# InternRobotics/InternNav

Measured on AMD Instinct MI355X. Metric: policy steps/sec/node, higher is better.
Workload: dtype bf16

## Files before the change

### internnav_amd/build.py

```python
from __future__ import annotations

import os
import subprocess
import sys
from concurrent.futures import ThreadPoolExecutor
from pathlib import Path

ROOT = Path(__file__).resolve().parent
CSRC = ROOT / "csrc"
OBJ = CSRC / "build"
LIB = ROOT / "libinternnav_amd.so"
ARCH = "gfx950"
FLAGS = ["-O3", "-std=c++17", "-fPIC", f"--offload-arch={ARCH}", "-fno-gpu-rdc", "-Wall", "-Wno-unused-function",
         "-ffp-contract=fast"]


def _sources():
    return sorted(list(CSRC.glob("*.hip")) + list(CSRC.glob("*.cpp")))


def _headers():
    return list(CSRC.glob("*.h")) + list((ROOT.parent / "include").glob("*.h"))


def _stale(target: Path, deps) -> bool:
    if not target.exists():
        return True
    t = target.stat().st_mtime
    return any(d.stat().st_mtime > t for d in deps)


def _compile(src: Path, verbose: bool) -> Path:
    obj = OBJ / (src.name + ".o")
    if _stale(obj, [src] + _headers()):
        cmd = ["hipcc", *FLAGS, "-x", "hip", "-c", str(src), "-o", str(obj)]
        if verbose:
            print(" ".join(cmd), flush=True)
        r = subprocess.run(cmd, capture_output=True, text=True)
        if r.returncode != 0:
            raise RuntimeError(f"hipcc failed for {src.name}:\n{r.stdout}\n{r.stderr}")
        if verbose and r.stderr.strip():
            print(r.stderr, file=sys.stderr)
    return obj


def build(verbose: bool = True) -> Path:
    OBJ.mkdir(parents=True, exist_ok=True)
    srcs = _sources()
    with ThreadPoolExecutor(max_workers=min(8, os.cpu_count() or 1)) as ex:
        objs = list(ex.map(lambda s: _compile(s, verbose), srcs))
    if _stale(LIB, objs):
        cmd = ["hipcc", "-shared", "-fPIC", f"--offload-arch={ARCH}", "-fno-gpu-rdc", *map(str, objs), "-o", str(LIB)]
        if verbose:
            print(" ".join(cmd), flush=True)
        r = subprocess.run(cmd, capture_output=True, text=True)
        if r.returncode != 0:
            raise RuntimeError(f"link failed:\n{r.stdout}\n{r.stderr}")
    return LIB


if __name__ == "__main__":
    print(build())
```

### internnav_amd/csrc/attention.hip

```cpp
#include "common.h"
#include "kernels.h"

namespace {

__device__ __forceinline__ int vt_pos(int kv_local) {
    int sub = kv_local >> 5, w = kv_local & 31;
    int t = w >> 4, x = w & 15;
    return (sub << 5) + ((x >> 2) << 3) + (x & 3) + (t << 2);
}

template <int DP, int DV, int NW, int KVB, bool DROP = false>
__global__ __launch_bounds__(NW * 64) void attn_fwd_kernel(AttnArgs p) {
    constexpr int NT = NW * 64;
    constexpr int KS_LD = DP + 8;
    constexpr int VT_LD = KVB + 8;
    constexpr int KCPR = DP / 8;
    constexpr int VCPR = DV / 8;
    constexpr int NKK = DP / 32;
    constexpr int NST = KVB / 16;
    constexpr int NSB = KVB / 32;
    constexpr int NDT = DV / 16;
    __shared__ __attribute__((aligned(16))) bf16 Ks[KVB * KS_LD];
    __shared__ __attribute__((aligned(16))) bf16 Vt[DV * VT_LD];

// ... 187 lines not shown
    f32x4 acc_o[NDT];
#pragma unroll
    for (int i = 0; i < NDT; ++i) acc_o[i] = f32x4{0.f, 0.f, 0.f, 0.f};
    if (kv0 < len_k) {
        bf16x8 qf[NKK];
#pragma unroll
        for (int kk = 0; kk < NKK; ++kk) {
            int d = kk * 32 + g * 8;
            qf[kk] = (live && d < p.D) ? *reinterpret_cast<const bf16x8*>(Q + d) : zero8;
        }
        constexpr int NKI = KVB * KCPR / 64, NVI = KVB * VCPR / 64;
        static_assert((KVB * KCPR) % 64 == 0 && (KVB * VCPR) % 64 == 0, "chunk pieces must divide evenly over the wave");
        bf16x8 kreg[NKI], vreg[NVI];
#pragma unroll
        for (int u = 0; u < NKI; ++u) {
            const int q = lane + u * 64, row = q / KCPR, c = q % KCPR, kv = kv0 + row;
            kreg[u] = (kv < len_k && c * 8 < p.D) ? *reinterpret_cast<const bf16x8*>(K + (size_t)kv * p.k_rs + c * 8) : zero8;
        }
#pragma unroll
        for (int u = 0; u < NVI; ++u) {
            const int q = lane + u * 64, row = q / VCPR, c = q % VCPR, kv = kv0 + row;
            vreg[u] = (kv < len_k) ? *reinterpret_cast<const bf16x8*>(V + (size_t)kv * p.v_rs + c * 8) : zero8;
        }
#pragma unroll
        for (int u = 0; u < NKI; ++u) {
            const int q = lane + u * 64, row = q / KCPR, c = q % KCPR;
            *reinterpret_cast<bf16x8*>(&Ks[row * KS_LD + c * 8]) = kreg[u];
        }
#pragma unroll
        for (int u = 0; u < NVI; ++u) {
            const int q = lane + u * 64, row = q / VCPR, c = q % VCPR;
            const int pos = vt_pos(row);
#pragma unroll
            for (int i = 0; i < 8; ++i) Vt[(c * 8 + i) * VT_LD + ((pos + 8 * c) & (KVB - 1))] = vreg[u][i];
        }
        __syncthreads();
        f32x4 s[NST];
#pragma unroll
        for (int t = 0; t < NST; ++t) {
            s[t] = f32x4{0.f, 0.f, 0.f, 0.f};
#pragma unroll
            for (int kk = 0; kk < NKK; ++kk) {
                bf16x8 kf = *reinterpret_cast<const bf16x8*>(&Ks[(t * 16 + lq) * KS_LD + kk * 32 + g * 8]);
                s[t] = __builtin_amdgcn_mfma_f32_16x16x32_bf16(kf, qf[kk], s[t], 0, 0, 0);
            }
        }
        const float sc = p.scale * 1.4426950408889634f;
        const int causal_shift = len_k - p.Lq;
        float mx = -INFINITY;
#pragma unroll
        for (int t = 0; t < NST; ++t)
#pragma unroll
            for (int r = 0; r < 4; ++r) {
                int kv = kv0 + t * 16 + g * 4 + r;
                bool ok = live && (kv < len_k) && (!p.causal || kv <= qpos + causal_shift);
                float v = ok ? s[t][r] * sc : -INFINITY;
                s[t][r] = v;
                mx = fmaxf(mx, v);
            }
        mx = fmaxf(mx, __shfl_xor(mx, 16));
        mx = fmaxf(mx, __shfl_xor(mx, 32));
        m_run = mx;
        const float m_use = (mx == -INFINITY) ? 0.f : mx;
        float rs = 0.f;
#pragma unroll
        for (int t = 0; t < NST; ++t)
#pragma unroll
            for (int r = 0; r < 4; ++r) {
                float e = exp2f(s[t][r] - m_use);
                s[t][r] = e;
                rs += e;
            }
        rs += __shfl_xor(rs, 16);
        rs += __shfl_xor(rs, 32);
        l_run = rs;
#pragma unroll
        for (int sb = 0; sb < NSB; ++sb) {
            bf16x8 pf;
#pragma unroll
            for (int r = 0; r < 4; ++r) {
                pf[r] = (bf16)s[2 * sb][r];
                pf[4 + r] = (bf16)s[2 * sb + 1][r];
            }
#pragma unroll
            for (int nt = 0; nt < NDT; ++nt) {
                bf16x8 vf = *reinterpret_cast<const bf16x8*>(&Vt[(nt * 16 + lq) * VT_LD + ((sb * 32 + g * 8 + 8 * ((nt * 16 + lq) >> 3)) & (KVB - 1))]);
                acc_o[nt] = __builtin_amdgcn_mfma_f32_16x16x32_bf16(vf, pf, acc_o[nt], 0, 0, 0);
            }
        }
    }
    float* orow = out + (size_t)lq * (DV + 2);
#pragma unroll
    for (int nt = 0; nt < NDT; ++nt) *reinterpret_cast<f32x4*>(orow + nt * 16 + g * 4) = acc_o[nt];
    if (g == 0) { orow[DV] = m_run; orow[DV + 1] = l_run; }
}

template <int DV>
__global__ __launch_bounds__(64) void attn_decode_combine_kernel(AttnArgs p, const float* __restrict__ ws, int nsplit, int rtiles) {
    const int lane = threadIdx.x;
    const int R = blockIdx.x, kh = blockIdx.y, b = blockIdx.z;
    const int G = p.H / p.Hkv;
    const int rt = R / 16, lq = R % 16;
    const int head = kh * G + R / p.Lq, qpos = R % p.Lq;
    const float* base = ws + (((size_t)b * p.Hkv + kh) * rtiles + rt) * nsplit * (size_t)(16 * (DV + 2)) + (size_t)lq * (DV + 2);
    const size_t sstride = (size_t)16 * (DV + 2);
    float m = -INFINITY;
    for (int s0 = 0; s0 < nsplit; s0 += 64) {
        const int s = s0 + lane;
        m = fmaxf(m, s < nsplit ? base[s * sstride + DV] : -INFINITY);
    }
    m = wave_max(m);
    const float m_use = (m == -INFINITY) ? 0.f : m;
    float l = 0.f, o0 = 0.f, o1 = 0.f;
    for (int s0 = 0; s0 < nsplit; s0 += 64) {
        const int s = s0 + lane;
        const float ms = s < nsplit ? base[s * sstride + DV] : -INFINITY;
        const float wl = (ms == -INFINITY) ? 0.f : exp2f(ms - m_use);
        l += s < nsplit ? base[s * sstride + DV + 1] * wl : 0.f;
        const int cnt = min(64, nsplit - s0);
#pragma unroll 8
        for (int j = 0; j < cnt; ++j) {
            const float w = __shfl(wl, j);
            const float* q = base + (size_t)(s0 + j) * sstride;
            if (lane < DV) o0 += q[lane] * w;
            if (lane + 64 < DV) o1 += q[lane + 64] * w;
        }
    }
    l = wave_sum(l);
    const float inv = l > 0.f ? 1.0f / l : 0.f;
    bf16* O = reinterpret_cast<bf16*>(p.O) + (size_t)b * p.o_bs + (size_t)qpos * p.o_rs + (size_t)head * p.o_hs;
    if (lane < p.D) O[lane] = (bf16)(o0 * inv);
    if (lane + 64 < p.D) O[lane + 64] = (bf16)(o1 * inv);
}

constexpr int DEC_FUSED_WAVES = 4, DEC_FUSED_MAX_CHUNKS = 16;

template <int DP, int DV>
__global__ __launch_bounds__(DEC_FUSED_WAVES * 64) void attn_decode_fused_kernel(AttnArgs p, int nsplit, int rtiles) {
    constexpr int KVB = 64, KS_LD = DP + 8, VT_LD = KVB + 8, KCPR = DP / 8, VCPR = DV / 8, NKK = DP / 32, NST = KVB / 16, NSB = KVB / 32, NDT = DV / 16;
    constexpr int PER_WAVE = KVB * KS_LD + DV * VT_LD;
    constexpr int PLD = DV + 2;
    static_assert(16 * PLD * 4 <= KVB * KS_LD * 2, "the partial of a wave fits its K image");
    extern __shared__ __attribute__((aligned(16))) char dec_smem[];
    const int tid = threadIdx.x, lane = tid & 63, g = lane >> 4, lq = lane & 15;
    const int wave = __builtin_amdgcn_readfirstlane(tid >> 6);
    bf16* Ks = reinterpret_cast<bf16*>(dec_smem) + wave * PER_WAVE;
    bf16* Vt = Ks + KVB * KS_LD;
    const int kh = blockIdx.x / rtiles, rt = blockIdx.x % rtiles, b = blockIdx.y;
    const int G = p.H / p.Hkv;
    const int R = rt * 16 + lq;
    const bool live = R < G * p.Lq;
    const int head = kh * G + (live ? R / p.Lq : 0), qpos = live ? R % p.Lq : 0;
    int len_k = p.Lk;
    if (p.k_len) len_k = min(p.k_len[b], p.Lk);
    const bf16* __restrict__ Q = reinterpret_cast<const bf16*>(p.Q) + (size_t)b * p.q_bs + (size_t)qpos * p.q_rs + (size_t)head * p.q_hs;
    const bf16* __restrict__ K = reinterpret_cast<const bf16*>(p.K) + (size_t)b * p.k_bs + (size_t)kh * p.k_hs;
    const bf16* __restrict__ V = reinterpret_cast<const bf16*>(p.V) + (size_t)b * p.v_bs + (size_t)kh * p.v_hs;
    const bf16x8 zero8 = {0, 0, 0, 0, 0, 0, 0, 0};
    float m_run = -INFINITY, l_run = 0.f;
    f32x4 acc_o[NDT];
#pragma unroll
    for (int i = 0; i < NDT; ++i) acc_o[i] = f32x4{0.f, 0.f, 0.f, 0.f};
    bf16x8 qf[NKK];
#pragma unroll
    for (int kk = 0; kk < NKK; ++kk) {
        const int d = kk * 32 + g * 8;
        qf[kk] = (live && d < p.D) ? *reinterpret_cast<const bf16x8*>(Q + d) : zero8;
    }
    constexpr int NKI = KVB * KCPR / 64, NVI = KVB * VCPR / 64;
    static_assert((KVB * KCPR) % 64 == 0 && (KVB * VCPR) % 64 == 0, "chunk pieces must divide evenly over the wave");
    bf16x8 kreg[NKI], vreg[NVI];
    auto fetch = [&](int kv0) {
#pragma unroll
        for (int u = 0; u < NKI; ++u) {
            const int q = lane + u * 64, row = q / KCPR, c = q % KCPR, kv = kv0 + row;
            kreg[u] = (kv < len_k && c * 8 < p.D) ? *reinterpret_cast<const bf16x8*>(K + (size_t)kv * p.k_rs + c * 8) : zero8;
        }
#pragma unroll
        for (int u = 0; u < NVI; ++u) {
            const int q = lane + u * 64, row = q / VCPR, c = q % VCPR, kv = kv0 + row;
            vreg[u] = (kv < len_k) ? *reinterpret_cast<const bf16x8*>(V + (size_t)kv * p.v_rs + c * 8) : zero8;
        }
    };
    const float sc = p.scale * 1.4426950408889634f;
    const int causal_shift = len_k - p.Lq;
    int split = wave;
    if (split * DEC_CHUNK < len_k) fetch(split * DEC_CHUNK);
    for (; split * DEC_CHUNK < len_k; split += DEC_FUSED_WAVES) {
        const int kv0 = split * DEC_CHUNK;
#pragma unroll
        for (int u = 0; u < NKI; ++u) {
            const int q = lane + u * 64, row = q / KCPR, c = q % KCPR;
            *reinterpret_cast<bf16x8*>(&Ks[row * KS_LD + c * 8]) = kreg[u];
        }
#pragma unroll
        for (int u = 0; u < NVI; ++u) {
            const int q = lane + u * 64, row = q / VCPR, c = q % VCPR;
            const int pos = vt_pos(row);
#pragma unroll
            for (int i = 0; i < 8; ++i) Vt[(c * 8 + i) * VT_LD + ((pos + 8 * c) & (KVB - 1))] = vreg[u][i];
        }
        if ((split + DEC_FUSED_WAVES) * DEC_CHUNK < len_k) fetch((split + DEC_FUSED_WAVES) * DEC_CHUNK);
        asm volatile("s_waitcnt lgkmcnt(0)" ::: "memory");
        __builtin_amdgcn_wave_barrier();
        f32x4 s[NST];
#pragma unroll
        for (int t = 0; t < NST; ++t) {
            s[t] = f32x4{0.f, 0.f, 0.f, 0.f};
#pragma unroll
            for (int kk = 0; kk < NKK; ++kk) {
                bf16x8 kf = *reinterpret_cast<const bf16x8*>(&Ks[(t * 16 + lq) * KS_LD + kk * 32 + g * 8]);
                s[t] = __builtin_amdgcn_mfma_f32_16x16x32_bf16(kf, qf[kk], s[t], 0, 0, 0);
            }
        }
        float mx = -INFINITY;
#pragma unroll
        for (int t = 0; t < NST; ++t)
#pragma unroll
            for (int r = 0; r < 4; ++r) {
                const int kv = kv0 + t * 16 + g * 4 + r;
                const bool ok = live && (kv < len_k) && (!p.causal || kv <= qpos + causal_shift);
                const float v = ok ? s[t][r] * sc : -INFINITY;
                s[t][r] = v;
                mx = fmaxf(mx, v);
            }
        mx = fmaxf(mx, __shfl_xor(mx, 16));
        mx = fmaxf(mx, __shfl_xor(mx, 32));
        const float m_new = fmaxf(m_run, mx);
        const float m_use = (m_new == -INFINITY) ? 0.f : m_new;
        const float alpha = (m_run == -INFINITY) ? 0.f : exp2f(m_run - m_use);
        float rs = 0.f;
#pragma unroll
        for (int t = 0; t < NST; ++t)
#pragma unroll
            for (int r = 0; r < 4; ++r) {
                const float e = exp2f(s[t][r] - m_use);
                s[t][r] = e;
                rs += e;
            }
        rs += __shfl_xor(rs, 16);
        rs += __shfl_xor(rs, 32);
        l_run = l_run * alpha + rs;
        m_run = m_new;
#pragma unroll
        for (int nt = 0; nt < NDT; ++nt)
#pragma unroll
            for (int r = 0; r < 4; ++r) acc_o[nt][r] *= alpha;
#pragma unroll
        for (int sb = 0; sb < NSB; ++sb) {
            bf16x8 pf;
#pragma unroll
            for (int r = 0; r < 4; ++r) {
                pf[r] = (bf16)s[2 * sb][r];
                pf[4 + r] = (bf16)s[2 * sb + 1][r];
            }
#pragma unroll
            for (int nt = 0; nt < NDT; ++nt) {
                bf16x8 vf = *reinterpret_cast<const bf16x8*>(&Vt[(nt * 16 + lq) * VT_LD + ((sb * 32 + g * 8 + 8 * ((nt * 16 + lq) >> 3)) & (KVB - 1))]);
                acc_o[nt] = __builtin_amdgcn_mfma_f32_16x16x32_bf16(vf, pf, acc_o[nt], 0, 0, 0);
            }
        }
    }
    asm volatile("s_waitcnt lgkmcnt(0)" ::: "memory");
    __builtin_amdgcn_wave_barrier();
    float* part = reinterpret_cast<float*>(Ks);
#pragma unroll
    for (int nt = 0; nt < NDT; ++nt) *reinterpret_cast<f32x4*>(part + lq * PLD + nt * 16 + g * 4) = acc_o[nt];
    if (g == 0) { part[lq * PLD + DV] = m_run; part[lq * PLD + DV + 1] = l_run; }
    __syncthreads();
    {
        constexpr int CPT = DV / 16;
        const int row = tid >> 4, c0 = (tid & 15) * CPT;
        const int Rr = rt * 16 + row;
        if (Rr < G * p.Lq) {
            const float* pw[DEC_FUSED_WAVES];
            float ms[DEC_FUSED_WAVES], m = -INFINITY;
#pragma unroll
            for (int w = 0; w < DEC_FUSED_WAVES; ++w) {
                pw[w] = reinterpret_cast<const float*>(reinterpret_cast<const bf16*>(dec_smem) + w * PER_WAVE) + row * PLD;
                ms[w] = pw[w][DV];
                m = fmaxf(m, ms[w]);
            }
            const float m_use = (m == -INFINITY) ? 0.f : m;
            float l = 0.f, o[CPT];
#pragma unroll
            for (int c = 0; c < CPT; ++c) o[c] = 0.f;
#pragma unroll
            for (int w = 0; w < DEC_FUSED_WAVES; ++w) {
                const float wl = (ms[w] == -INFINITY) ? 0.f : exp2f(ms[w] - m_use);
                l += pw[w][DV + 1] * wl;
#pragma unroll
                for (int c = 0; c < CPT; ++c) o[c] += pw[w][c0 + c] * wl;
            }
            const float inv = l > 0.f ? 1.0f / l : 0.f;
            const int hd = kh * G + Rr / p.Lq, qp = Rr % p.Lq;
            bf16* O = reinterpret_cast<bf16*>(p.O) + (size_t)b * p.o_bs + (size_t)qp * p.o_rs + (size_t)hd * p.o_hs;
#pragma unroll
            for (int c = 0; c < CPT; ++c)
                if (c0 + c < p.D) O[c0 + c] = (bf16)(o[c] * inv);
        }
    }
}

constexpr int DEC8_WAVES = 8;

template <int DP, int DV>
__global__ __launch_bounds__(DEC8_WAVES * 64) void attn_decode_fused8_kernel(AttnArgs p, int nsplit, int rtiles) {
    constexpr int KVB = 64, VT_LD = KVB + 8, VCPR = DV / 8, NKK = DP / 32, NST = KVB / 16, NSB = KVB / 32, NDT = DV / 16, HDT = NDT / 2, DH = DV / 2;
    constexpr int PER_WAVE = DH * VT_LD;
    constexpr int PLD = DV + 2;
    static_assert(16 * PLD * 4 <= PER_WAVE * 2, "the partial of a wave fits its V^T image");
    static_assert(NDT % 2 == 0 && VCPR % 2 == 0, "the head dim splits into two halves of whole 16-column tiles");
    extern __shared__ __attribute__((aligned(16))) char dec_smem[];
    const int tid = threadIdx.x, lane = tid & 63, g = lane >> 4, lq = lane & 15;
    const int wave = __builtin_amdgcn_readfirstlane(tid >> 6);
    bf16* Vt = reinterpret_cast<bf16*>(dec_smem) + wave * PER_WAVE;
    const int kh = blockIdx.x / rtiles, rt = blockIdx.x % rtiles, b = blockIdx.y;
    const int G = p.H / p.Hkv;
    const int R = rt * 16 + lq;
    const bool live = R < G * p.Lq;
    const int head = kh * G + (live ? R / p.Lq : 0), qpos = live ? R % p.Lq : 0;
    int len_k = p.Lk;
    if (p.k_len) len_k = min(p.k_len[b], p.Lk);
    const bf16* __restrict__ Q = reinterpret_cast<const bf16*>(p.Q) + (size_t)b * p.q_bs + (size_t)qpos * p.q_rs + (size_t)head * p.q_hs;
    const bf16* __restrict__ K = reinterpret_cast<const bf16*>(p.K) + (size_t)b * p.k_bs + (size_t)kh * p.k_hs;
    const bf16* __restrict__ V = reinterpret_cast<const bf16*>(p.V) + (size_t)b * p.v_bs + (size_t)kh * p.v_hs;
    const bf16x8 zero8 = {0, 0, 0, 0, 0, 0, 0, 0};
    float m_run = -INFINITY, l_run = 0.f;
    f32x4 acc_o[NDT];
#pragma unroll
    for (int i = 0; i < NDT; ++i) acc_o[i] = f32x4{0.f, 0.f, 0.f, 0.f};
    bf16x8 qf[NKK];
#pragma unroll
    for (int kk = 0; kk < NKK; ++kk) {
        const int d = kk * 32 + g * 8;
        qf[kk] = (live && d < p.D) ? *reinterpret_cast<const bf16x8*>(Q + d) : zero8;
    }
    if constexpr (DP == 128 && DV == 128) {
        if (p.rope_cos) {
            if (live) {
                const float* cr = p.rope_cos + ((size_t)b * p.Lq + qpos) * DP + g * 8;
                const float* sr = p.rope_sin + ((size_t)b * p.Lq + qpos) * DP + g * 8;
#pragma unroll
                for (int kk = 0; kk < NKK / 2; ++kk) {
                    const bf16x8 lo = qf[kk], hi = qf[kk + NKK / 2];
                    bf16x8 olo, ohi;
#pragma unroll
                    for (int i = 0; i < 8; ++i) {
                        const int d = kk * 32 + i;
                        olo[i] = (bf16)ina_rope_lo((float)lo[i], (float)hi[i], cr[d], sr[d]);
                        ohi[i] = (bf16)ina_rope_hi((float)lo[i], (float)hi[i], cr[d + DP / 2], sr[d + DP / 2]);
                    }
                    qf[kk] = olo;
                    qf[kk + NKK / 2] = ohi;
                }
            }
            for (int r = wave >> 1; r < p.Lq; r += DEC8_WAVES / 2) {
                const size_t src = (size_t)b * p.kn_bs + (size_t)r * p.kn_rs + (size_t)kh * p.kn_hs;
                const size_t row = (size_t)(len_k - p.Lq + r);
                if ((wave & 1) == 0) {
                    if (lane < 8) {
                        const bf16* kn = reinterpret_cast<const bf16*>(p.k_new) + src + lane * 8;
                        const bf16x8 lo = *reinterpret_cast<const bf16x8*>(kn), hi = *reinterpret_cast<const bf16x8*>(kn + DP / 2);
                        const float* cr = p.rope_cos + ((size_t)b * p.Lq + r) * DP + lane * 8;
                        const float* sr = p.rope_sin + ((size_t)b * p.Lq + r) * DP + lane * 8;
                        bf16x8 olo, ohi;
#pragma unroll
                        for (int i = 0; i < 8; ++i) {
                            olo[i] = (bf16)ina_rope_lo((float)lo[i], (float)hi[i], cr[i], sr[i]);
                            ohi[i] = (bf16)ina_rope_hi((float)lo[i], (float)hi[i], cr[i + DP / 2], sr[i + DP / 2]);
                        }
                        bf16* kd = const_cast<bf16*>(K) + row * p.k_rs + lane * 8;
                        *reinterpret_cast<bf16x8*>(kd) = olo;
                        *reinterpret_cast<bf16x8*>(kd + DP / 2) = ohi;
                    }
                } else if (lane < 16) {
                    *reinterpret_cast<bf16x8*>(const_cast<bf16*>(V) + row * p.v_rs + lane * 8) =
                        *reinterpret_cast<const bf16x8*>(reinterpret_cast<const bf16*>(p.v_new) + src + lane * 8);
                }
            }
            asm volatile("s_waitcnt vmcnt(0)" ::: "memory");
            __syncthreads();
        }
    }
    constexpr int NVI = KVB * VCPR / 64;
    static_assert((KVB * VCPR) % 64 == 0, "chunk pieces must divide evenly over the wave");
    bf16x8 kf[NST][NKK], vreg[NVI];
    auto fetch = [&](int kv0) {
#pragma unroll
        for (int t = 0; t < NST; ++t) {
            const int kv = kv0 + t * 16 + lq;
            const bf16* kr = K + (size_t)(kv < len_k ? kv : len_k - 1) * p.k_rs + g * 8;
#pragma unroll
            for (int kk = 0; kk < NKK; ++kk) kf[t][kk] = (kk * 32 + g * 8 < p.D) ? *reinterpret_cast<const bf16x8*>(kr + kk * 32) : zero8;
        }
#pragma unroll
        for (int u = 0; u < NVI; ++u) {
            const int q = lane + u * 64, row = q / VCPR, c = q % VCPR, kv = kv0 + row;
            vreg[u] = (kv < len_k) ? *reinterpret_cast<const bf16x8*>(V + (size_t)kv * p.v_rs + c * 8) : zero8;
        }
    };
    const float sc = p.scale * 1.4426950408889634f;
    const int causal_shift = len_k - p.Lq;
    const int vc = lane % VCPR;
    int split = wave;
    if (split * DEC_CHUNK < len_k) fetch(split * DEC_CHUNK);
    for (; split * DEC_CHUNK < len_k; split += DEC8_WAVES) {
        const int kv0 = split * DEC_CHUNK;
        f32x4 s[NST];
#pragma unroll
        for (int t = 0; t < NST; ++t) {
            s[t] = f32x4{0.f, 0.f, 0.f, 0.f};
#pragma unroll
            for (int kk = 0; kk < NKK; ++kk) s[t] = __builtin_amdgcn_mfma_f32_16x16x32_bf16(kf[t][kk], qf[kk], s[t], 0, 0, 0);
        }
        bf16x8 vcur[NVI];
#pragma unroll
        for (int u = 0; u < NVI; ++u) vcur[u] = vreg[u];
        float mx = -INFINITY;
#pragma unroll
        for (int t = 0; t < NST; ++t)
#pragma unroll
            for (int r = 0; r < 4; ++r) {
                const int kv = kv0 + t * 16 + g * 4 + r;
                const bool ok = live && (kv < len_k) && (!p.causal || kv <= qpos + causal_shift);
                const float v = ok ? s[t][r] * sc : -INFINITY;
                s[t][r] = v;
                mx = fmaxf(mx, v);
            }
        mx = fmaxf(mx, __shfl_xor(mx, 16));
        mx = fmaxf(mx, __shfl_xor(mx, 32));
        const float m_new = fmaxf(m_run, mx);
        const float m_use = (m_new == -INFINITY) ? 0.f : m_new;
        const float alpha = (m_run == -INFINITY) ? 0.f : exp2f(m_run - m_use);
        float rs = 0.f;
#pragma unroll
        for (int t = 0; t < NST; ++t)
#pragma unroll
            for (int r = 0; r < 4; ++r) {
                const float e = exp2f(s[t][r] - m_use);
                s[t][r] = e;
                rs += e;
            }
        rs += __shfl_xor(rs, 16);
        rs += __shfl_xor(rs, 32);
        l_run = l_run * alpha + rs;
        m_run = m_new;
#pragma unroll
        for (int nt = 0; nt < NDT; ++nt)
#pragma unroll
            for (int r = 0; r < 4; ++r) acc_o[nt][r] *= alpha;
        bf16x8 pf[NSB];
#pragma unroll
        for (int sb = 0; sb < NSB; ++sb)
#pragma unroll
            for (int r = 0; r < 4; ++r) {
                pf[sb][r] = (bf16)s[2 * sb][r];
                pf[sb][4 + r] = (bf16)s[2 * sb + 1][r];
            }
#pragma unroll
        for (int hv = 0; hv < 2; ++hv) {
            if (vc / (VCPR / 2) == hv) {
#pragma unroll
                for (int u = 0; u < NVI; ++u) {
                    const int row = (lane + u * 64) / VCPR;
                    const int pos = vt_pos(row);
#pragma unroll
                    for (int i = 0; i < 8; ++i) Vt[((vc - hv * (VCPR / 2)) * 8 + i) * VT_LD + ((pos + 8 * vc) & (KVB - 1))] = vcur[u][i];
                }
            }
            if (hv == 1 && (split + DEC8_WAVES) * DEC_CHUNK < len_k) fetch((split + DEC8_WAVES) * DEC_CHUNK);
            asm volatile("s_waitcnt lgkmcnt(0)" ::: "memory");
            __builtin_amdgcn_wave_barrier();
#pragma unroll
            for (int sb = 0; sb < NSB; ++sb)
#pragma unroll
                for (int n2 = 0; n2 < HDT; ++n2) {
                    const int dl = n2 * 16 + lq, d = hv * DH + dl;
                    const bf16x8 vf = *reinterpret_cast<const bf16x8*>(&Vt[dl * VT_LD + ((sb * 32 + g * 8 + 8 * (d >> 3)) & (KVB - 1))]);
                    acc_o[hv * HDT + n2] = __builtin_amdgcn_mfma_f32_16x16x32_bf16(vf, pf[sb], acc_o[hv * HDT + n2], 0, 0, 0);
                }
        }
    }
    asm volatile("s_waitcnt lgkmcnt(0)" ::: "memory");
    __builtin_amdgcn_wave_barrier();
    float* part = reinterpret_cast<float*>(Vt);
#pragma unroll
    for (int nt = 0; nt < NDT; ++nt) *reinterpret_cast<f32x4*>(part + lq * PLD + nt * 16 + g * 4) = acc_o[nt];
    if (g == 0) { part[lq * PLD + DV] = m_run; part[lq * PLD + DV + 1] = l_run; }
    __syncthreads();
    if (tid < 256) {
        constexpr int CPT = DV / 16;
        const int row = tid >> 4, c0 = (tid & 15) * CPT;
        const int Rr = rt * 16 + row;
        if (Rr < G * p.Lq) {
            float m = -INFINITY;
#pragma unroll
            for (int w = 0; w < DEC8_WAVES; ++w)
                m = fmaxf(m, (reinterpret_cast<const float*>(reinterpret_cast<const bf16*>(dec_smem) + w * PER_WAVE) + row * PLD)[DV]);
            const float m_use = (m == -INFINITY) ? 0.f : m;
            float l = 0.f, o[CPT];
#pragma unroll
            for (int c = 0; c < CPT; ++c) o[c] = 0.f;
#pragma unroll
            for (int w = 0; w < DEC8_WAVES; ++w) {
                const float* pw = reinterpret_cast<const float*>(reinterpret_cast<const bf16*>(dec_smem) + w * PER_WAVE) + row * PLD;
                const float ms = pw[DV];
                const float wl = (ms == -INFINITY) ? 0.f : exp2f(ms - m_use);
                l += pw[DV + 1] * wl;
#pragma unroll
                for (int c = 0; c < CPT; ++c) o[c] += pw[c0 + c] * wl;
            }
            const float inv = l > 0.f ? 1.0f / l : 0.f;
            const int hd = kh * G + Rr / p.Lq, qp = Rr % p.Lq;
            bf16* O = reinterpret_cast<bf16*>(p.O) + (size_t)b * p.o_bs + (size_t)qp * p.o_rs + (size_t)hd * p.o_hs;
#pragma unroll
            for (int c = 0; c < CPT; ++c)
                if (c0 + c < p.D) O[c0 + c] = (bf16)(o[c] * inv);
        }
    }
}

template <int DP, int DV>
int launch_decode(const AttnArgs& p, hipStream_t stream) {
    const int G = p.H / p.Hkv;
    const int rtiles = (G * p.Lq + 15) / 16;
    const int nsplit = (p.Lk + DEC_CHUNK - 1) / DEC_CHUNK;
    const double keys = p.causal ? 0.5 * ((double)p.Lk + (double)(p.Lk - p.Lq) + 1.0) : (double)p.Lk;
    InaProfScope prof(INA_PROF_ATTN, 4.0 * p.B * p.H * (double)p.Lq * keys * p.D,
                      2.0 * p.D * ((double)p.B * p.H * p.Lq * 2.0 + 2.0 * (double)p.B * p.Hkv * p.Lk), stream);
    if constexpr (DV == 128 && DP == 128) {
        if (nsplit <= DEC_FUSED_MAX_CHUNKS && p.kernel != 1 && p.kernel != 3) {
            INA_REQUIRE(!p.rope_cos || (p.rope_sin && p.k_new && p.v_new && p.D == 128 && p.causal && p.kn_rs % 8 == 0 && p.kn_hs % 8 == 0 && p.kn_bs % 8 == 0 &&
                                        ((uintptr_t)p.k_new % 16) == 0 && ((uintptr_t)p.v_new % 16) == 0 && p.k_rs % 8 == 0 && p.v_rs % 8 == 0),
                        "attention(rope): needs rope_sin, k_new, v_new, d = 128, causal decode and 16-byte aligned rows");
            constexpr size_t LDS8 = (size_t)DEC8_WAVES * (DV / 2) * (64 + 8) * sizeof(bf16);
            auto kern8 = attn_decode_fused8_kernel<DP, DV>;
            static bool attr8_done = false;
            if (!attr8_done) {
                INA_HIP_CHECK(hipFuncSetAttribute(reinterpret_cast<const void*>(kern8), hipFuncAttributeMaxDynamicSharedMemorySize, (int)LDS8));
                attr8_done = true;
            }
            hipLaunchKernelGGL(kern8, dim3(p.Hkv * rtiles, p.B), dim3(DEC8_WAVES * 64), LDS8, stream, p, nsplit, rtiles);
            INA_HIP_CHECK(hipGetLastError());
            return 0;
        }
    }
    if (nsplit <= DEC_FUSED_MAX_CHUNKS && p.kernel != 1) {
        constexpr size_t LDS = (size_t)DEC_FUSED_WAVES * (64 * (DP + 8) + DV * (64 + 8)) * sizeof(bf16);
        auto kern = attn_decode_fused_kernel<DP, DV>;
        static bool attr_done = false;
        if (!attr_done) {
            INA_HIP_CHECK(hipFuncSetAttribute(reinterpret_cast<const void*>(kern), hipFuncAttributeMaxDynamicSharedMemorySize, (int)LDS));
            attr_done = true;
        }
        hipLaunchKernelGGL(kern, dim3(p.Hkv * rtiles, p.B), dim3(DEC_FUSED_WAVES * 64), LDS, stream, p, nsplit, rtiles);
        INA_HIP_CHECK(hipGetLastError());
        return 0;
    }
    const size_t bytes = (size_t)p.B * p.Hkv * rtiles * nsplit * 16 * (DV + 2) * sizeof(float);
    float* ws = nullptr;
    if (int rc = ina_workspace(1, bytes, stream, &ws)) return rc;
    hipLaunchKernelGGL((attn_decode_split_kernel<DP, DV>), dim3(nsplit, p.Hkv * rtiles, p.B), dim3(64), 0, stream, p, ws, nsplit, rtiles);
    hipLaunchKernelGGL((attn_decode_combine_kernel<DV>), dim3(G * p.Lq, p.Hkv, p.B), dim3(64), 0, stream, p, ws, nsplit, rtiles);
    INA_HIP_CHECK(hipGetLastError());
    return 0;
}

template <int DP, int DV>
int launch_d(const AttnArgs& p, hipStream_t stream) {
    if (!p.cu_q && !p.cu_k && p.kv_bdiv == 1 && p.kv_start == 0 && !p.accumulate && !p.head_gate && !p.drop_thresh && p.Lk >= 256 &&
        (p.H / p.Hkv) * p.Lq <= 48 && p.Lq <= 8 && DV <= 128)
        return launch_decode<DP, DV>(p, stream);
    const bool small_k = p.Lk <= 48;
    int nw = (p.Lq <= 16) ? 1 : (p.Lq <= 32 ? 2 : 4);
    dim3 grid((p.Lq + nw * 16 - 1) / (nw * 16), p.H, p.B);
    const double keys = p.causal ? 0.5 * ((double)p.Lk + (double)(p.Lk - p.Lq) + 1.0) : (double)(p.Lk - p.kv_start);
    InaProfScope prof(INA_PROF_ATTN, 4.0 * p.B * p.H * (double)p.Lq * keys * p.D,
                      2.0 * p.D * ((double)p.B * p.H * p.Lq * 2.0 + 2.0 * (double)(p.B / p.kv_bdiv) * p.Hkv * p.Lk), stream);
    INA_REQUIRE(p.kernel != 3, "attention: kernel = 3 (the four-wave one-launch decode kernel) outside the decode contract (few query rows, dense K / V, Lk >= 256)");
    if (p.kernel == 2) INA_REQUIRE(ina_attention_wide_contract(p), "attention: kernel = 2 (32-rows-per-wave) outside its contract (d 64 / 80 / 128, Lq, Lk >= 128, no gate / accumulate / dropout)");
    if (p.kernel == 2 || (p.kernel == 0 && ina_attention_wide_eligible(p)))
        return ina_launch_attention_wide(p, stream);
    if (p.drop_thresh) {
        if constexpr (DP <= 64) {
#define INA_ATTN_LAUNCH_DROP(NW_, KVB_) \
    hipLaunchKernelGGL((attn_fwd_kernel<DP, DV, NW_, KVB_, true>), grid, dim3(NW_ * 64), 0, stream, p)
            if (nw == 1) { if (small_k) INA_ATTN_LAUNCH_DROP(1, 32); else INA_ATTN_LAUNCH_DROP(1, 64); }
            else if (nw == 2) { if (small_k) INA_ATTN_LAUNCH_DROP(2, 32); else INA_ATTN_LAUNCH_DROP(2, 64); }
            else { if (small_k) INA_ATTN_LAUNCH_DROP(4, 32); else INA_ATTN_LAUNCH_DROP(4, 64); }
#undef INA_ATTN_LAUNCH_DROP
            INA_HIP_CHECK(hipGetLastError());
            return 0;
        } else {
            ina_set_error("attention: dropout is built for head dims <= 64 only");
            return -2;
        }
    }
#define INA_ATTN_LAUNCH(NW_, KVB_) \
    hipLaunchKernelGGL((attn_fwd_kernel<DP, DV, NW_, KVB_>), grid, dim3(NW_ * 64), 0, stream, p)
    if (nw == 1) { if (small_k) INA_ATTN_LAUNCH(1, 32); else INA_ATTN_LAUNCH(1, 64); }
    else if (nw == 2) { if (small_k) INA_ATTN_LAUNCH(2, 32); else INA_ATTN_LAUNCH(2, 64); }
    else { if (small_k) INA_ATTN_LAUNCH(4, 32); else INA_ATTN_LAUNCH(4, 64); }
#undef INA_ATTN_LAUNCH
    INA_HIP_CHECK(hipGetLastError());
    return 0;
}

}

int ina_launch_attention(const AttnArgs& p_in, hipStream_t stream) {
    AttnArgs p = p_in;
    if (p.kv_bdiv <= 0) p.kv_bdiv = 1;
    INA_REQUIRE(p.B > 0 && p.H > 0 && p.Hkv > 0 && p.H % p.Hkv == 0, "attention: bad B/H/Hkv (%d,%d,%d)", p.B, p.H, p.Hkv);
    INA_REQUIRE(p.Lq > 0 && p.Lk > 0, "attention: empty sequence Lq=%d Lk=%d", p.Lq, p.Lk);
    INA_REQUIRE(p.q_rs % 8 == 0 && p.k_rs % 8 == 0 && p.v_rs % 8 == 0 && p.o_rs % 4 == 0 && p.q_hs % 8 == 0 && p.k_hs % 8 == 0 &&
                    p.v_hs % 8 == 0 && p.o_hs % 4 == 0 && p.q_bs % 8 == 0 && p.k_bs % 8 == 0 && p.v_bs % 8 == 0 && p.o_bs % 4 == 0,
                "attention: strides must keep 16-byte row alignment");
    INA_REQUIRE(((uintptr_t)p.Q % 16) == 0 && ((uintptr_t)p.K % 16) == 0 && ((uintptr_t)p.V % 16) == 0 && ((uintptr_t)p.O % 8) == 0,
                "attention: misaligned pointer");
    if (p.rope_cos) {
        const bool decode = !p.cu_q && !p.cu_k && p.kv_bdiv == 1 && p.kv_start == 0 && !p.accumulate && !p.head_gate && !p.drop_thresh && p.Lk >= 256 &&
                            (p.H / p.Hkv) * p.Lq <= 48 && p.Lq <= 8;
        INA_REQUIRE(decode && p.D == 128 && (p.Lk + DEC_CHUNK - 1) / DEC_CHUNK <= DEC_FUSED_MAX_CHUNKS && p.kernel == 0,
                    "attention(rope): the fused rotary embedding + KV append needs the one-launch decode kernel (d = 128, 256 <= Lk <= %d, Lq <= 8, kernel 0): Lq=%d Lk=%d D=%d",
                    DEC_CHUNK * DEC_FUSED_MAX_CHUNKS, p.Lq, p.Lk, p.D);
    }
    switch (p.D) {
        case 48: return launch_d<64, 48>(p, stream);
        case 64: return launch_d<64, 64>(p, stream);
        case 80: return launch_d<96, 80>(p, stream);
        case 128: return launch_d<128, 128>(p, stream);
        default: ina_set_error("attention: unsupported head dim %d (48/64/80/128)", p.D); return -2;
    }
}
```

Measured before the change: 301.8.

## Replace 8-wave fused decode attention with 16-wave head-dim-split kernel

Replaces the 8-wave decode attention kernel with a 16-wave kernel where each wave handles one 64-key chunk, with no loop or online rescaling. The head dimension is split across 2 or 4 sibling blocks so the grid has more blocks when batch times heads is small. Rotary embedding of Q and new K is spread across all threads and staged in LDS, and the KV-cache append is done only by one block per group. The kernel also accepts kernel=4 for any Lk. In exchange, K and Q work is repeated in every sibling block, the chunk count is capped at 16 per block, and a build-time early-return skip is added.

```diff
diff --git a/internnav_amd/build.py b/internnav_amd/build.py
--- a/internnav_amd/build.py
+++ b/internnav_amd/build.py
@@ -45,8 +45,10 @@
 
 
 def build(verbose: bool = True) -> Path:
+    srcs = _sources()
+    if not _stale(LIB, srcs + _headers()):
+        return LIB
     OBJ.mkdir(parents=True, exist_ok=True)
-    srcs = _sources()
     with ThreadPoolExecutor(max_workers=min(8, os.cpu_count() or 1)) as ex:
         objs = list(ex.map(lambda s: _compile(s, verbose), srcs))
     if _stale(LIB, objs):
diff --git a/internnav_amd/csrc/attention.hip b/internnav_amd/csrc/attention.hip
--- a/internnav_amd/csrc/attention.hip
+++ b/internnav_amd/csrc/attention.hip
@@ -513,20 +513,25 @@
     }
 }
 
-constexpr int DEC8_WAVES = 8;
-
-template <int DP, int DV>
-__global__ __launch_bounds__(DEC8_WAVES * 64) void attn_decode_fused8_kernel(AttnArgs p, int nsplit, int rtiles) {
-    constexpr int KVB = 64, VT_LD = KVB + 8, VCPR = DV / 8, NKK = DP / 32, NST = KVB / 16, NSB = KVB / 32, NDT = DV / 16, HDT = NDT / 2, DH = DV / 2;
-    constexpr int PER_WAVE = DH * VT_LD;
-    constexpr int PLD = DV + 2;
-    static_assert(16 * PLD * 4 <= PER_WAVE * 2, "the partial of a wave fits its V^T image");
-    static_assert(NDT % 2 == 0 && VCPR % 2 == 0, "the head dim splits into two halves of whole 16-column tiles");
+constexpr int DECW_WAVES = 16, DECW_PASS = 32;
+
+template <int DSPLIT>
+__global__ __launch_bounds__(DECW_WAVES * 64) void attn_decode_wide_kernel(AttnArgs p, int rtiles, int ngroups, int gpad) {
+    constexpr int D = 128, KVB = 64, VT_LD = KVB + 8, NKK = D / 32, NST = KVB / 16, NSB = KVB / 32;
+    constexpr int DW = D / DSPLIT, NDT = DW / 16, NPASS = DW / DECW_PASS, VC = DW / 8;
+    constexpr int PER_WAVE = DECW_PASS * VT_LD;
+    constexpr int PLD = DW + 4, PART = 16 * PLD;
+    static_assert(DW % DECW_PASS == 0 && 64 % VC == 0 && KVB == DEC_CHUNK, "whole image passes; a lane keeps one piece column");
+    static_assert((DECW_WAVES * PART + DECW_WAVES * 32) * 4 <= DECW_WAVES * PER_WAVE * 2, "the partials fit the images they overlay");
+    static_assert(16 * DW <= DECW_WAVES * 64, "one output element per thread");
     extern __shared__ __attribute__((aligned(16))) char dec_smem[];
     const int tid = threadIdx.x, lane = tid & 63, g = lane >> 4, lq = lane & 15;
     const int wave = __builtin_amdgcn_readfirstlane(tid >> 6);
+    const int sib = blockIdx.x / gpad, grp = blockIdx.x % gpad;
+    if (grp >= ngroups) return;
+    const int b = grp / (p.Hkv * rtiles), kh = (grp / rtiles) % p.Hkv, rt = grp % rtiles;
+    const int d0 = sib * DW;
     bf16* Vt = reinterpret_cast<bf16*>(dec_smem) + wave * PER_WAVE;
-    const int kh = blockIdx.x / rtiles, rt = blockIdx.x % rtiles, b = blockIdx.y;
     const int G = p.H / p.Hkv;
     const int R = rt * 16 + lq;
     const bool live = R < G * p.Lq;
@@ -534,90 +539,114 @@
     int len_k = p.Lk;
     if (p.k_len) len_k = min(p.k_len[b], p.Lk);
     const bf16* __restrict__ Q = reinterpret_cast<const bf16*>(p.Q) + (size_t)b * p.q_bs + (size_t)qpos * p.q_rs + (size_t)head * p.q_hs;
-    const bf16* __restrict__ K = reinterpret_cast<const bf16*>(p.K) + (size_t)b * p.k_bs + (size_t)kh * p.k_hs;
-    const bf16* __restrict__ V = reinterpret_cast<const bf16*>(p.V) + (size_t)b * p.v_bs + (size_t)kh * p.v_hs;
+    const bf16* K = reinterpret_cast<const bf16*>(p.K) + (size_t)b * p.k_bs + (size_t)kh * p.k_hs;
+    const bf16* V = reinterpret_cast<const bf16*>(p.V) + (size_t)b * p.v_bs + (size_t)kh * p.v_hs;
     const bf16x8 zero8 = {0, 0, 0, 0, 0, 0, 0, 0};
+    const bool rope = p.rope_cos != nullptr;
+    const int new0 = rope ? len_k - p.Lq : len_k;
+    const int kv0 = wave * KVB;
+    const bool active = kv0 < len_k;
     float m_run = -INFINITY, l_run = 0.f;
     f32x4 acc_o[NDT];
 #pragma unroll
     for (int i = 0; i < NDT; ++i) acc_o[i] = f32x4{0.f, 0.f, 0.f, 0.f};
-    bf16x8 qf[NKK];
-#pragma unroll
-    for (int kk = 0; kk < NKK; ++kk) {
-        const int d = kk * 32 + g * 8;
-        qf[kk] = (live && d < p.D) ? *reinterpret_cast<const bf16x8*>(Q + d) : zero8;
-    }
-    if constexpr (DP == 128 && DV == 128) {
-        if (p.rope_cos) {
-            if (live) {
-                const float* cr = p.rope_cos + ((size_t)b * p.Lq + qpos) * DP + g * 8;
-                const float* sr = p.rope_sin + ((size_t)b * p.Lq + qpos) * DP + g * 8;
-#pragma unroll
-                for (int kk = 0; kk < NKK / 2; ++kk) {
-                    const bf16x8 lo = qf[kk], hi = qf[kk + NKK / 2];
-                    bf16x8 olo, ohi;
-#pragma unroll
-                    for (int i = 0; i < 8; ++i) {
-                        const int d = kk * 32 + i;
-                        olo[i] = (bf16)ina_rope_lo((float)lo[i], (float)hi[i], cr[d], sr[d]);
-                        ohi[i] = (bf16)ina_rope_hi((float)lo[i], (float)hi[i], cr[d + DP / 2], sr[d + DP / 2]);
+
+    constexpr int QS_LD = D + 8;
+    bf16* qs = reinterpret_cast<bf16*>(dec_smem);
+    bf16* ks = qs + 16 * QS_LD;
+    static_assert((16 + 8) * QS_LD <= 2 * PER_WAVE, "rotated q / new keys sit inside the first two images");
+    const bool appender = sib == 0 && rt == 0;
+    bf16x2 r_lo = {0, 0}, r_hi = {0, 0};
+    f32x2 r_cl = {0.f, 0.f}, r_ch = r_cl, r_sl = r_cl, r_sh = r_cl;
+    bf16x8 r_v = zero8;
+    bool r_on = false;
+    const int r_row = tid < 512 ? tid >> 5 : tid < 768 ? (tid - 512) >> 5 : (tid - 768) >> 4;
+    const int r_j = (tid & 31) * 2;
+    if (rope && tid < 896) {
+        const bool isq = tid < 512;
+        const int Rq = rt * 16 + r_row;
+        r_on = isq ? Rq < G * p.Lq : (r_row < p.Lq && len_k - p.Lq + r_row >= 0);
+        const int tok = !r_on ? 0 : isq ? Rq % p.Lq : r_row;
+        const size_t knew = (size_t)b * p.kn_bs + (size_t)tok * p.kn_rs + (size_t)kh * p.kn_hs;
+        if (tid < 768) {
+            const bf16* src = isq ? reinterpret_cast<const bf16*>(p.Q) + (size_t)b * p.q_bs + (size_t)tok * p.q_rs + (size_t)(kh * G + (r_on ? Rq / p.Lq : 0)) * p.q_hs + r_j
+                                  : reinterpret_cast<const bf16*>(p.k_new) + knew + r_j;
+            const float* cr = p.rope_cos + ((size_t)b * p.Lq + tok) * D + r_j;
+            const float* sr = p.rope_sin + ((size_t)b * p.Lq + tok) * D + r_j;
+            r_lo = *reinterpret_cast<const bf16x2*>(src); r_hi = *reinterpret_cast<const bf16x2*>(src + D / 2);
+            r_cl = *reinterpret_cast<const f32x2*>(cr); r_ch = *reinterpret_cast<const f32x2*>(cr + D / 2);
+            r_sl = *reinterpret_cast<const f32x2*>(sr); r_sh = *reinterpret_cast<const f32x2*>(sr + D / 2);
+        } else if (appender) {
+            r_v = *reinterpret_cast<const bf16x8*>(reinterpret_cast<const bf16*>(p.v_new) + knew + (tid & 15) * 8);
+        }
+    }
+
+    bf16x8 kf[NST][NKK], vreg[VC], qf[NKK];
+    const int vc = lane % VC;
+    if (active) {
+        if (!rope) {
+#pragma unroll
+            for (int kk = 0; kk < NKK; ++kk) qf[kk] = *reinterpret_cast<const bf16x8*>(Q + kk * 32 + g * 8);
+        }
+#pragma unroll
+        for (int t = 0; t < NST; ++t) {
+            const bf16* kr = K + (size_t)min(kv0 + t * 16 + lq, len_k - 1) * p.k_rs + g * 8;
+#pragma unroll
+            for (int kk = 0; kk < NKK; ++kk) kf[t][kk] = *reinterpret_cast<const bf16x8*>(kr + kk * 32);
+        }
+#pragma unroll
+        for (int u = 0; u < VC; ++u) {
+            const int kv = kv0 + (lane + u * 64) / VC;
+            const bool nw = kv >= new0 && kv < len_k;
+            const bf16* vr = nw ? reinterpret_cast<const bf16*>(p.v_new) + (size_t)b * p.kn_bs + (size_t)(kv - new0) * p.kn_rs + (size_t)kh * p.kn_hs
+                                : V + (size_t)min(kv, len_k - 1) * p.v_rs;
+            vreg[u] = *reinterpret_cast<const bf16x8*>(vr + d0 + vc * 8);
+        }
+    }
+    if (rope) {
+        if (tid < 768) {
+            bf16x2 olo, ohi;
+#pragma unroll
+            for (int i = 0; i < 2; ++i) {
+                olo[i] = (bf16)ina_rope_lo((float)r_lo[i], (float)r_hi[i], r_cl[i], r_sl[i]);
+                ohi[i] = (bf16)ina_rope_hi((float)r_lo[i], (float)r_hi[i], r_ch[i], r_sh[i]);
+            }
+            if (!r_on) { olo = bf16x2{0, 0}; ohi = olo; }
+            bf16* dst = (tid < 512 ? qs : ks) + r_row * QS_LD + r_j;
+            *reinterpret_cast<bf16x2*>(dst) = olo;
+            *reinterpret_cast<bf16x2*>(dst + D / 2) = ohi;
+            if (tid >= 512 && r_on && appender) {
+                bf16* kd = const_cast<bf16*>(K) + (size_t)(len_k - p.Lq + r_row) * p.k_rs + r_j;
+                *reinterpret_cast<bf16x2*>(kd) = olo;
+                *reinterpret_cast<bf16x2*>(kd + D / 2) = ohi;
+            }
+        } else if (tid < 896 && appender && r_on) {
+            *reinterpret_cast<bf16x8*>(const_cast<bf16*>(V) + (size_t)(len_k - p.Lq + r_row) * p.v_rs + (tid & 15) * 8) = r_v;
+        }
+        __syncthreads();
+        if (active) {
+#pragma unroll
+            for (int kk = 0; kk < NKK; ++kk) qf[kk] = *reinterpret_cast<const bf16x8*>(qs + lq * QS_LD + kk * 32 + g * 8);
+            if (kv0 + KVB > new0) {
+#pragma unroll
+                for (int t = 0; t < NST; ++t) {
+                    const int kv = kv0 + t * 16 + lq;
+                    if (kv >= new0 && kv < len_k) {
+#pragma unroll
+                        for (int kk = 0; kk < NKK; ++kk) kf[t][kk] = *reinterpret_cast<const bf16x8*>(ks + (kv - new0) * QS_LD + kk * 32 + g * 8);
                     }
-                    qf[kk] = olo;
-                    qf[kk + NKK / 2] = ohi;
                 }
             }
-            for (int r = wave >> 1; r < p.Lq; r += DEC8_WAVES / 2) {
-                const size_t src = (size_t)b * p.kn_bs + (size_t)r * p.kn_rs + (size_t)kh * p.kn_hs;
-                const size_t row = (size_t)(len_k - p.Lq + r);
-                if ((wave & 1) == 0) {
-                    if (lane < 8) {
-                        const bf16* kn = reinterpret_cast<const bf16*>(p.k_new) + src + lane * 8;
-                        const bf16x8 lo = *reinterpret_cast<const bf16x8*>(kn), hi = *reinterpret_cast<const bf16x8*>(kn + DP / 2);
-                        const float* cr = p.rope_cos + ((size_t)b * p.Lq + r) * DP + lane * 8;
-                        const float* sr = p.rope_sin + ((size_t)b * p.Lq + r) * DP + lane * 8;
-                        bf16x8 olo, ohi;
-#pragma unroll
-                        for (int i = 0; i < 8; ++i) {
-                            olo[i] = (bf16)ina_rope_lo((float)lo[i], (float)hi[i], cr[i], sr[i]);
-                            ohi[i] = (bf16)ina_rope_hi((float)lo[i], (float)hi[i], cr[i + DP / 2], sr[i + DP / 2]);
-                        }
-                        bf16* kd = const_cast<bf16*>(K) + row * p.k_rs + lane * 8;
-                        *reinterpret_cast<bf16x8*>(kd) = olo;
-                        *reinterpret_cast<bf16x8*>(kd + DP / 2) = ohi;
-                    }
-                } else if (lane < 16) {
-                    *reinterpret_cast<bf16x8*>(const_cast<bf16*>(V) + row * p.v_rs + lane * 8) =
-                        *reinterpret_cast<const bf16x8*>(reinterpret_cast<const bf16*>(p.v_new) + src + lane * 8);
-                }
-            }
-            asm volatile("s_waitcnt vmcnt(0)" ::: "memory");
-            __syncthreads();
-        }
-    }
-    constexpr int NVI = KVB * VCPR / 64;
-    static_assert((KVB * VCPR) % 64 == 0, "chunk pieces must divide evenly over the wave");
-    bf16x8 kf[NST][NKK], vreg[NVI];
-    auto fetch = [&](int kv0) {
-#pragma unroll
-        for (int t = 0; t < NST; ++t) {
-            const int kv = kv0 + t * 16 + lq;
-            const bf16* kr = K + (size_t)(kv < len_k ? kv : len_k - 1) * p.k_rs + g * 8;
-#pragma unroll
-            for (int kk = 0; kk < NKK; ++kk) kf[t][kk] = (kk * 32 + g * 8 < p.D) ? *reinterpret_cast<const bf16x8*>(kr + kk * 32) : zero8;
-        }
-#pragma unroll
-        for (int u = 0; u < NVI; ++u) {
-            const int q = lane + u * 64, row = q / VCPR, c = q % VCPR, kv = kv0 + row;
-            vreg[u] = (kv < len_k) ? *reinterpret_cast<const bf16x8*>(V + (size_t)kv * p.v_rs + c * 8) : zero8;
-        }
-    };
-    const float sc = p.scale * 1.4426950408889634f;
-    const int causal_shift = len_k - p.Lq;
-    const int vc = lane % VCPR;
-    int split = wave;
-    if (split * DEC_CHUNK < len_k) fetch(split * DEC_CHUNK);
-    for (; split * DEC_CHUNK < len_k; split += DEC8_WAVES) {
-        const int kv0 = split * DEC_CHUNK;
+        }
+        asm volatile("s_waitcnt lgkmcnt(0)" ::: "memory");
+        __syncthreads();
+    }
+
+    if (active) {
+        if (!live) {
+#pragma unroll
+            for (int kk = 0; kk < NKK; ++kk) qf[kk] = zero8;
+        }
         f32x4 s[NST];
 #pragma unroll
         for (int t = 0; t < NST; ++t) {
@@ -625,9 +654,8 @@
 #pragma unroll
             for (int kk = 0; kk < NKK; ++kk) s[t] = __builtin_amdgcn_mfma_f32_16x16x32_bf16(kf[t][kk], qf[kk], s[t], 0, 0, 0);
         }
-        bf16x8 vcur[NVI];
-#pragma unroll
-        for (int u = 0; u < NVI; ++u) vcur[u] = vreg[u];
+        const float sc = p.scale * 1.4426950408889634f;
+        const int causal_shift = len_k - p.Lq;
         float mx = -INFINITY;
 #pragma unroll
         for (int t = 0; t < NST; ++t)
@@ -641,9 +669,8 @@
             }
         mx = fmaxf(mx, __shfl_xor(mx, 16));
         mx = fmaxf(mx, __shfl_xor(mx, 32));
-        const float m_new = fmaxf(m_run, mx);
-        const float m_use = (m_new == -INFINITY) ? 0.f : m_new;
-        const float alpha = (m_run == -INFINITY) ? 0.f : exp2f(m_run - m_use);
+        m_run = mx;
+        const float m_use = (mx == -INFINITY) ? 0.f : mx;
         float rs = 0.f;
 #pragma unroll
         for (int t = 0; t < NST; ++t)
@@ -655,12 +682,7 @@
             }
         rs += __shfl_xor(rs, 16);
         rs += __shfl_xor(rs, 32);
-        l_run = l_run * alpha + rs;
-        m_run = m_new;
-#pragma unroll
-        for (int nt = 0; nt < NDT; ++nt)
-#pragma unroll
-            for (int r = 0; r < 4; ++r) acc_o[nt][r] *= alpha;
+        l_run = rs;
         bf16x8 pf[NSB];
 #pragma unroll
         for (int sb = 0; sb < NSB; ++sb)
@@ -670,64 +692,54 @@
                 pf[sb][4 + r] = (bf16)s[2 * sb + 1][r];
             }
 #pragma unroll
-        for (int hv = 0; hv < 2; ++hv) {
-            if (vc / (VCPR / 2) == hv) {
-#pragma unroll
-                for (int u = 0; u < NVI; ++u) {
-                    const int row = (lane + u * 64) / VCPR;
-                    const int pos = vt_pos(row);
-#pragma unroll
-                    for (int i = 0; i < 8; ++i) Vt[((vc - hv * (VCPR / 2)) * 8 + i) * VT_LD + ((pos + 8 * vc) & (KVB - 1))] = vcur[u][i];
+        for (int hv = 0; hv < NPASS; ++hv) {
+            if (vc / (DECW_PASS / 8) == hv) {
+#pragma unroll
+                for (int u = 0; u < VC; ++u) {
+                    const int pos = vt_pos((lane + u * 64) / VC);
+                    const bf16x8 x = kv0 + (lane + u * 64) / VC < len_k ? vreg[u] : zero8;
+#pragma unroll
+                    for (int i = 0; i < 8; ++i) Vt[((vc - hv * (DECW_PASS / 8)) * 8 + i) * VT_LD + ((pos + 8 * vc) & (KVB - 1))] = x[i];
                 }
             }
-            if (hv == 1 && (split + DEC8_WAVES) * DEC_CHUNK < len_k) fetch((split + DEC8_WAVES) * DEC_CHUNK);
             asm volatile("s_waitcnt lgkmcnt(0)" ::: "memory");
             __builtin_amdgcn_wave_barrier();
 #pragma unroll
             for (int sb = 0; sb < NSB; ++sb)
 #pragma unroll
-                for (int n2 = 0; n2 < HDT; ++n2) {
-                    const int dl = n2 * 16 + lq, d = hv * DH + dl;
-                    const bf16x8 vf = *reinterpret_cast<const bf16x8*>(&Vt[dl * VT_LD + ((sb * 32 + g * 8 + 8 * (d >> 3)) & (KVB - 1))]);
-                    acc_o[hv * HDT + n2] = __builtin_amdgcn_mfma_f32_16x16x32_bf16(vf, pf[sb], acc_o[hv * HDT + n2], 0, 0, 0);
+                for (int n2 = 0; n2 < DECW_PASS / 16; ++n2) {
+                    const int dl = n2 * 16 + lq, dloc = hv * DECW_PASS + dl;
+                    const bf16x8 vf = *reinterpret_cast<const bf16x8*>(&Vt[dl * VT_LD + ((sb * 32 + g * 8 + 8 * (dloc >> 3)) & (KVB - 1))]);
+                    acc_o[hv * (DECW_PASS / 16) + n2] = __builtin_amdgcn_mfma_f32_16x16x32_bf16(vf, pf[sb], acc_o[hv * (DECW_PASS / 16) + n2], 0, 0, 0);
                 }
         }
     }
-    asm volatile("s_waitcnt lgkmcnt(0)" ::: "memory");
-    __builtin_amdgcn_wave_barrier();
-    float* part = reinterpret_cast<float*>(Vt);
-#pragma unroll
-    for (int nt = 0; nt < NDT; ++nt) *reinterpret_cast<f32x4*>(part + lq * PLD + nt * 16 + g * 4) = acc_o[nt];
-    if (g == 0) { part[lq * PLD + DV] = m_run; part[lq * PLD + DV + 1] = l_run; }
     __syncthreads();
-    if (tid < 256) {
-        constexpr int CPT = DV / 16;
-        const int row = tid >> 4, c0 = (tid & 15) * CPT;
+    float* parts = reinterpret_cast<float*>(dec_smem);
+    float* stats = parts + DECW_WAVES * PART;
+#pragma unroll
+    for (int nt = 0; nt < NDT; ++nt) *reinterpret_cast<f32x4*>(parts + wave * PART + lq * PLD + nt * 16 + g * 4) = acc_o[nt];
+    if (g == 0) { stats[(wave * 16 + lq) * 2] = m_run; stats[(wave * 16 + lq) * 2 + 1] = l_run; }
+    __syncthreads();
+    if (tid < 16 * DW) {
+        const int row = tid / DW, col = tid % DW;
         const int Rr = rt * 16 + row;
         if (Rr < G * p.Lq) {
             float m = -INFINITY;
 #pragma unroll
-            for (int w = 0; w < DEC8_WAVES; ++w)
-                m = fmaxf(m, (reinterpret_cast<const float*>(reinterpret_cast<const bf16*>(dec_smem) + w * PER_WAVE) + row * PLD)[DV]);
+            for (int w = 0; w < DECW_WAVES; ++w) m = fmaxf(m, stats[(w * 16 + row) * 2]);
             const float m_use = (m == -INFINITY) ? 0.f : m;
-            float l = 0.f, o[CPT];
-#pragma unroll
-            for (int c = 0; c < CPT; ++c) o[c] = 0.f;
-#pragma unroll
-            for (int w = 0; w < DEC8_WAVES; ++w) {
-                const float* pw = reinterpret_cast<const float*>(reinterpret_cast<const bf16*>(dec_smem) + w * PER_WAVE) + row * PLD;
-                const float ms = pw[DV];
+            float l = 0.f, o = 0.f;
+#pragma unroll
+            for (int w = 0; w < DECW_WAVES; ++w) {
+                const float ms = stats[(w * 16 + row) * 2];
                 const float wl = (ms == -INFINITY) ? 0.f : exp2f(ms - m_use);
-                l += pw[DV + 1] * wl;
-#pragma unroll
-                for (int c = 0; c < CPT; ++c) o[c] += pw[c0 + c] * wl;
+                l += stats[(w * 16 + row) * 2 + 1] * wl;
+                o += parts[w * PART + row * PLD + col] * wl;
             }
             const float inv = l > 0.f ? 1.0f / l : 0.f;
             const int hd = kh * G + Rr / p.Lq, qp = Rr % p.Lq;
-            bf16* O = reinterpret_cast<bf16*>(p.O) + (size_t)b * p.o_bs + (size_t)qp * p.o_rs + (size_t)hd * p.o_hs;
-#pragma unroll
-            for (int c = 0; c < CPT; ++c)
-                if (c0 + c < p.D) O[c0 + c] = (bf16)(o[c] * inv);
+            reinterpret_cast<bf16*>(p.O)[(size_t)b * p.o_bs + (size_t)qp * p.o_rs + (size_t)hd * p.o_hs + d0 + col] = (bf16)(o * inv);
         }
     }
 }
@@ -745,18 +757,22 @@
             INA_REQUIRE(!p.rope_cos || (p.rope_sin && p.k_new && p.v_new && p.D == 128 && p.causal && p.kn_rs % 8 == 0 && p.kn_hs % 8 == 0 && p.kn_bs % 8 == 0 &&
                                         ((uintptr_t)p.k_new % 16) == 0 && ((uintptr_t)p.v_new % 16) == 0 && p.k_rs % 8 == 0 && p.v_rs % 8 == 0),
                         "attention(rope): needs rope_sin, k_new, v_new, d = 128, causal decode and 16-byte aligned rows");
-            constexpr size_t LDS8 = (size_t)DEC8_WAVES * (DV / 2) * (64 + 8) * sizeof(bf16);
-            auto kern8 = attn_decode_fused8_kernel<DP, DV>;
-            static bool attr8_done = false;
-            if (!attr8_done) {
-                INA_HIP_CHECK(hipFuncSetAttribute(reinterpret_cast<const void*>(kern8), hipFuncAttributeMaxDynamicSharedMemorySize, (int)LDS8));
-                attr8_done = true;
-            }
-            hipLaunchKernelGGL(kern8, dim3(p.Hkv * rtiles, p.B), dim3(DEC8_WAVES * 64), LDS8, stream, p, nsplit, rtiles);
+            constexpr size_t LDSW = (size_t)DECW_WAVES * DECW_PASS * (64 + 8) * sizeof(bf16);
+            const int ngroups = p.B * p.Hkv * rtiles, gpad = (ngroups + 7) / 8 * 8;
+            const bool four = ngroups * 4 <= 256;
+            auto kernw = four ? attn_decode_wide_kernel<4> : attn_decode_wide_kernel<2>;
+            static bool attrw_done = false;
+            if (!attrw_done) {
+                INA_HIP_CHECK(hipFuncSetAttribute(reinterpret_cast<const void*>(attn_decode_wide_kernel<4>), hipFuncAttributeMaxDynamicSharedMemorySize, (int)LDSW));
+                INA_HIP_CHECK(hipFuncSetAttribute(reinterpret_cast<const void*>(attn_decode_wide_kernel<2>), hipFuncAttributeMaxDynamicSharedMemorySize, (int)LDSW));
+                attrw_done = true;
+            }
+            hipLaunchKernelGGL(kernw, dim3(gpad * (four ? 4 : 2)), dim3(DECW_WAVES * 64), LDSW, stream, p, rtiles, ngroups, gpad);
             INA_HIP_CHECK(hipGetLastError());
             return 0;
         }
     }
+    INA_REQUIRE(p.kernel != 4, "attention: kernel = 4 (the 16-wave one-launch decode kernel) needs d = 128 and Lk <= %d", DEC_CHUNK * DEC_FUSED_MAX_CHUNKS);
     if (nsplit <= DEC_FUSED_MAX_CHUNKS && p.kernel != 1) {
         constexpr size_t LDS = (size_t)DEC_FUSED_WAVES * (64 * (DP + 8) + DV * (64 + 8)) * sizeof(bf16);
         auto kern = attn_decode_fused_kernel<DP, DV>;
@@ -780,8 +796,8 @@
 
 template <int DP, int DV>
 int launch_d(const AttnArgs& p, hipStream_t stream) {
-    if (!p.cu_q && !p.cu_k && p.kv_bdiv == 1 && p.kv_start == 0 && !p.accumulate && !p.head_gate && !p.drop_thresh && p.Lk >= 256 &&
-        (p.H / p.Hkv) * p.Lq <= 48 && p.Lq <= 8 && DV <= 128)
+    if (!p.cu_q && !p.cu_k && p.kv_bdiv == 1 && p.kv_start == 0 && !p.accumulate && !p.head_gate && !p.drop_thresh &&
+        (p.Lk >= 256 || p.kernel == 3 || p.kernel == 4) && (p.H / p.Hkv) * p.Lq <= 48 && p.Lq <= 8 && DV <= 128)
         return launch_decode<DP, DV>(p, stream);
     const bool small_k = p.Lk <= 48;
     int nw = (p.Lq <= 16) ? 1 : (p.Lq <= 32 ? 2 : 4);
@@ -789,7 +805,7 @@
     const double keys = p.causal ? 0.5 * ((double)p.Lk + (double)(p.Lk - p.Lq) + 1.0) : (double)(p.Lk - p.kv_start);
     InaProfScope prof(INA_PROF_ATTN, 4.0 * p.B * p.H * (double)p.Lq * keys * p.D,
                       2.0 * p.D * ((double)p.B * p.H * p.Lq * 2.0 + 2.0 * (double)(p.B / p.kv_bdiv) * p.Hkv * p.Lk), stream);
-    INA_REQUIRE(p.kernel != 3, "attention: kernel = 3 (the four-wave one-launch decode kernel) outside the decode contract (few query rows, dense K / V, Lk >= 256)");
+    INA_REQUIRE(p.kernel != 3 && p.kernel != 4, "attention: kernel = %d (a pinned one-launch decode kernel) outside the decode contract (few query rows, dense K / V)", p.kernel);
     if (p.kernel == 2) INA_REQUIRE(ina_attention_wide_contract(p), "attention: kernel = 2 (32-rows-per-wave) outside its contract (d 64 / 80 / 128, Lq, Lk >= 128, no gate / accumulate / dropout)");
     if (p.kernel == 2 || (p.kernel == 0 && ina_attention_wide_eligible(p)))
         return ina_launch_attention_wide(p, stream);
@@ -831,10 +847,10 @@
     INA_REQUIRE(((uintptr_t)p.Q % 16) == 0 && ((uintptr_t)p.K % 16) == 0 && ((uintptr_t)p.V % 16) == 0 && ((uintptr_t)p.O % 8) == 0,
                 "attention: misaligned pointer");
     if (p.rope_cos) {
-        const bool decode = !p.cu_q && !p.cu_k && p.kv_bdiv == 1 && p.kv_start == 0 && !p.accumulate && !p.head_gate && !p.drop_thresh && p.Lk >= 256 &&
-                            (p.H / p.Hkv) * p.Lq <= 48 && p.Lq <= 8;
-        INA_REQUIRE(decode && p.D == 128 && (p.Lk + DEC_CHUNK - 1) / DEC_CHUNK <= DEC_FUSED_MAX_CHUNKS && p.kernel == 0,
-                    "attention(rope): the fused rotary embedding + KV append needs the one-launch decode kernel (d = 128, 256 <= Lk <= %d, Lq <= 8, kernel 0): Lq=%d Lk=%d D=%d",
+        const bool decode = !p.cu_q && !p.cu_k && p.kv_bdiv == 1 && p.kv_start == 0 && !p.accumulate && !p.head_gate && !p.drop_thresh &&
+                            (p.H / p.Hkv) * p.Lq <= 48 && p.Lq <= 8 && p.Lq <= p.Lk;
+        INA_REQUIRE(decode && p.D == 128 && (p.Lk + DEC_CHUNK - 1) / DEC_CHUNK <= DEC_FUSED_MAX_CHUNKS && ((p.kernel == 0 && p.Lk >= 256) || p.kernel == 4),
+                    "attention(rope): the fused rotary embedding + KV append needs the one-launch decode kernel (d = 128, 256 <= Lk <= %d - any Lk with kernel 4 -, Lq <= 8, kernel 0 / 4): Lq=%d Lk=%d D=%d",
                     DEC_CHUNK * DEC_FUSED_MAX_CHUNKS, p.Lq, p.Lk, p.D);
     }
     switch (p.D) {
```

Result: no change. 303.1 (median of 6 runs) (+0.4%).
